# CODEJIN/GST_Tacotron

Measured on AMD Instinct MI355X. Metric: mel-frames/s, higher is better.
Workload: dtype f32; 1 GPU; BASELINE configs[1]: GST on, batch 32 per GPU, 128-token utterances, Step_Reduction 2, Max_Step 1000, LJSpeech 80-mel hparams; whole Inference_Step (encoder+GST+decode+postnet, vocoder excluded); global_batch=32, ref_frames=256, parallelism=utterance-sharded x1 + final RCCL gather, gather=none (one rank)

## Files before the change

gst_tacotron_amd/capi.py:

```python
import ctypes
import os

import numpy as np
import torch

from .hparams import Dims

_HERE = os.path.dirname(os.path.abspath(__file__))
LIB_PATH = os.path.join(_HERE, "lib", "libgsttaco.so")

MAX_LAYERS = 8
ABI_VERSION = 13
ATT_CODES = {"BMA": 0, "SMA": 1, "LSA": 2}

EXPORTED_SYMBOLS = (
    "gsttaco_abi_version", "gsttaco_create", "gsttaco_destroy", "gsttaco_last_error",
    "gsttaco_num_weights", "gsttaco_weight_info", "gsttaco_load_weight", "gsttaco_finalize_weights",
    "gsttaco_encode", "gsttaco_gst", "gsttaco_decode", "gsttaco_postnet", "gsttaco_vocoder", "gsttaco_inference_step",
    "gsttaco_mel_frontend", "gsttaco_mel_basis", "gsttaco_griffin_lim", "gsttaco_crc32c",
    "gsttaco_set_profiling", "gsttaco_get_profile", "gsttaco_lstm_launch_bytes", "gsttaco_debug_stamps", "gsttaco_decode_plan", "gsttaco_debug_randomness",
    "gsttaco_set_graph_policy", "gsttaco_graph_cache_size", "gsttaco_debug_handoff_error", "gsttaco_debug_raise_handoff_error", "gsttaco_debug_counters",
    "gsttaco_synchronize", "gsttaco_debug_conv_prepare", "gsttaco_debug_conv_run",
)

CONV_V = {
    "IG_1411": 0, "IG_2212": 1, "IG_2222": 2, "IG_4113": 3, "IG_4112": 4, "IG_4111": 5,
    "C2D_1411": 6, "C2D_4112": 7, "C2D_4111": 8,
    "WINO4": 9, "WINO2": 10, "WINO4_S": 11, "WINO2_S": 12, "WINO4_S_X3": 13, "WINO2_S_X3": 14,
    "GEMM_SPLIT": 15,
    "C5_RN4": 16, "C5_RN4_XB": 17, "C5_RN4_OB": 18, "C5_RN4_XB_OB": 19,
    "C5_RN2": 20, "C5_RN2_XB": 21, "C5_RN2_OB": 22, "C5_RN2_XB_OB": 23,
    "BF16_RM2": 24, "BF16_RM2_XB": 25, "BF16_RM2_OB": 26, "BF16_RM2_XB_OB": 27,
    "BF16_RM1": 28, "BF16_RM1_XB": 29, "BF16_RM1_OB": 30, "BF16_RM1_XB_OB": 31,
}
CONV_V_INVALID = -1
CONV_V_NAMES = {v: k for k, v in CONV_V.items()}
CONV_FORM = {"FP32": 1, "BF16": 2, "WINO2": 4, "WINO4": 8, "WINO_SPLIT": 16, "GEMM_SPLIT": 32}
# ... 78 lines not shown
    lib.gsttaco_decode.argtypes = [vp, vp, vp, vp, vp, vp, u64, i32, i32, i32, vp, vp, vp, vp]
    lib.gsttaco_postnet.argtypes = [vp, vp, i32, i32, vp, vp]
    lib.gsttaco_vocoder.argtypes = [vp, vp, i32, i32, vp, vp]
    lib.gsttaco_inference_step.argtypes = [vp, vp, vp, vp, vp, vp, vp, u64, i32, i32, i32, i32, vp, vp, vp, vp, vp, vp]
    lib.gsttaco_mel_frontend.argtypes = [vp, vp, vp, i32, i32, ctypes.c_float, vp, vp, i32, vp]
    lib.gsttaco_mel_basis.argtypes = [vp, f32p]
    lib.gsttaco_griffin_lim.argtypes = [vp, vp, vp, i32, i32, i32, ctypes.c_float, ctypes.c_float, vp, u64, vp, vp, i32, vp]
    lib.gsttaco_set_profiling.argtypes = [vp, i32]
    lib.gsttaco_get_profile.argtypes = [vp, i32, ctypes.POINTER(ctypes.c_float), ctypes.POINTER(ctypes.c_int)]
    lib.gsttaco_lstm_launch_bytes.argtypes = [vp, i32, i32]
    lib.gsttaco_lstm_launch_bytes.restype = ctypes.c_int64
    lib.gsttaco_debug_stamps.argtypes = [vp, ctypes.POINTER(ctypes.c_uint64)]
    lib.gsttaco_debug_stamps.restype = ctypes.c_int
    lib.gsttaco_decode_plan.argtypes = [vp, i32, ctypes.POINTER(ctypes.c_int32)]
    lib.gsttaco_decode_plan.restype = ctypes.c_int
    lib.gsttaco_debug_randomness.argtypes = [vp, vp, vp, i32, i32, i32]
    lib.gsttaco_debug_randomness.restype = ctypes.c_int
    lib.gsttaco_set_graph_policy.argtypes = [vp, i32, i32]
    lib.gsttaco_set_graph_policy.restype = ctypes.c_int
    lib.gsttaco_graph_cache_size.argtypes = [vp]
    lib.gsttaco_graph_cache_size.restype = ctypes.c_int
    lib.gsttaco_debug_handoff_error.argtypes = [vp, ctypes.POINTER(ctypes.c_uint32)]
    lib.gsttaco_debug_handoff_error.restype = ctypes.c_int
    lib.gsttaco_debug_raise_handoff_error.argtypes = [vp, ctypes.c_uint32]
    lib.gsttaco_debug_raise_handoff_error.restype = ctypes.c_int
    lib.gsttaco_debug_counters.argtypes = [vp, ctypes.POINTER(ctypes.c_uint64)]
    lib.gsttaco_debug_counters.restype = ctypes.c_int
    lib.gsttaco_synchronize.argtypes = [vp, vp]
    lib.gsttaco_synchronize.restype = ctypes.c_int
    lib.gsttaco_debug_conv_prepare.argtypes = [vp, ctypes.POINTER(ConvDesc), f32p, f32p, f32p, ctypes.POINTER(ctypes.c_int)]
# ... 116 lines not shown
```

gst_tacotron_amd/csrc/gsttaco.cpp:

```cpp
#include <hip/hip_runtime.h>

#include <algorithm>
#include <atomic>
#include <cmath>
#include <cstdio>
#include <cstdlib>
#include <cstring>
#include <map>
#include <mutex>
#include <string>
#include <vector>

#include "../../include/gsttaco.h"
#include "kernels.h"

namespace {

constexpr float kBnEps = 1e-3f;

struct HostTensor {
    std::string name;
    std::vector<int64_t> shape;
    std::vector<float> data;
    bool loaded = false;
// ... 2399 lines not shown
    }
    const uint8_t* p = static_cast<const uint8_t*>(data);
    uint32_t c = crc ^ 0xffffffffu;
    while (n >= 8) {
        uint32_t lo, hi;
        memcpy(&lo, p, 4); memcpy(&hi, p + 4, 4);
        lo ^= c;
        c = tab[7][lo & 0xff] ^ tab[6][(lo >> 8) & 0xff] ^ tab[5][(lo >> 16) & 0xff] ^ tab[4][lo >> 24] ^
            tab[3][hi & 0xff] ^ tab[2][(hi >> 8) & 0xff] ^ tab[1][(hi >> 16) & 0xff] ^ tab[0][hi >> 24];
        p += 8; n -= 8;
    }
    while (n--) c = tab[0][(c ^ *p++) & 0xff] ^ (c >> 8);
    return c ^ 0xffffffffu;
}

int gsttaco_debug_randomness(gsttaco_ctx* c, float* host_masks, float* host_noise, int steps, int B, int Tv) {
    if (!c || steps < 1 || B < 1 || Tv < 1 || steps > c->steps_max || B > c->cfg.max_batch || Tv > c->cfg.max_tokens)
        return GSTTACO_E_INVALID;
    HIPCHECK(c, hipDeviceSynchronize());
    if (host_masks && c->masks_lazy) {
        HIPCHECK(c, gt_launch_rng_fill(c->w_seed, c->w_masks, nullptr, steps, B, c->P0, c->P1, Tv, c->cfg.prenet_rate, nullptr));
        HIPCHECK(c, hipDeviceSynchronize());
    }
    if (host_masks && c->dec_padded) {
        float* tmp = nullptr;
        const size_t n = (size_t)steps * B * (c->P0t + c->P1t);
        HIPCHECK(c, hipMalloc((void**)&tmp, n * 4));
        hipError_t e = gt_launch_relayout_masks(c->w_masks, tmp, steps, B, c->P0t, c->P1t, c->P0, c->P1, 0, nullptr);
        if (e == hipSuccess) e = hipMemcpy(host_masks, tmp, n * 4, hipMemcpyDeviceToHost);
        (void)hipFree(tmp);
// ... 116 lines not shown
```

gst_tacotron_amd/csrc/kernels.h:

```cpp
#pragma once
#include <hip/hip_runtime.h>
#include <stdint.h>

enum { EPI_LINEAR = 0, EPI_RELU_DROP = 1, EPI_LSTM = 2, EPI_PARTIAL = 3 };

struct SkinnySeg {
    const float* ptr;
    int64_t ld;
    int nkb;
    int blocked;
};
__host__ __device__ inline size_t gt_blk_off(int row, int k, int MT) {
    return (((size_t)(k >> 4) * MT + (row >> 4)) << 8) + (size_t)(((((k & 15) >> 2) << 4) + (row & 15)) * 4 + (k & 3));
}

__host__ __device__ inline size_t gt_blk_off_h(int row, int k, int MT) {
    return ((((size_t)(k >> 5) * MT + (row >> 4)) << 6) + (size_t)((((k & 15) >> 2) << 4) + (row & 15))) * 8 + (size_t)((((k >> 4) & 1) << 2) + (k & 3));
}

struct SkinnyArgs {
    const float* wp;
    const float* bias;
    SkinnySeg seg[3];
    int nkb;
// ... 256 lines not shown
    float* hpart;
    float* stash;
    uint32_t* ctl;
    uint32_t* err;
    float* pre; int64_t ld_pre;
    float* stop;
    float* align; int64_t ld_align;
    int B, MT, Tv, steps, co_tiles;
    int G, n_chain, tvp, twopass;
    int expect_extra;
    unsigned long long* dbg;
};
size_t gt_persist_decode_ctl_words();
bool gt_persist_decode_supported(int mel, int r, int P0, int P1, int A, int H1, int H2, int B, int Tv, int pj_tiles, int pj_nkb, int slots, int bf16);
int gt_persist_decode_max_batch();
bool gt_persist_decode_lsa_fits(int B, int Tv, int loc_f, int loc_k);
hipError_t gt_persist_decode_init();
int gt_persist_decode_blocks_per_cu();
hipError_t gt_launch_persist_decode(const PersistDecodeArgs& a, const float* b0, hipStream_t stream);

struct Conv2dArgs {
    const float* x;
    int64_t xb;
    const float* w;
    const float* scale;
    const float* shift;
    float* out;
    int B, H, W, Cin, Cout, Ho, Wo, k, stride, pad_h, pad_w;
};
hipError_t gt_launch_conv2d_bn_relu(const Conv2dArgs& a, hipStream_t stream);
// ... 59 lines not shown
```

gst_tacotron_amd/csrc/persist_decode.hip:

```cpp
#include "chain_common.h"
#include "device_utils.h"
#include "kernels.h"
#include "../../include/gsttaco.h"

namespace {

constexpr int PD_NT = 512, PD_NW = 8, PD_NWG = 256, PD_UTT = 32, PD_HELP = 64;
constexpr int PD_P = 256, PD_A = 128, PD_H = 1024, PD_TVMAX = 256, PD_LDV = PD_A + 4;
constexpr int PD_GMAX = 4, PD_BMAX = 32 * PD_GMAX;
constexpr int PD_KBP = PD_P / 16, PD_KBC = PD_A / 16, PD_KBH = PD_H / 16, PD_KBPJ = PD_KBH + PD_KBC;
constexpr uint32_t PD_SPIN_MAX = 1u << 20;

#ifndef PD_FS
#define PD_FS 16
#endif
#ifndef PD_SLEEP_N
#define PD_SLEEP_N 0
#endif
#define PD_SLEEP() do { if (PD_SLEEP_N > 0) __builtin_amdgcn_s_sleep(PD_SLEEP_N); } while (0)
#define PD_ZT(zt) int zt = 0; asm volatile("" : "+v"(zt))
#ifndef PD_X2_EARLY
#define PD_X2_EARLY 1
#endif
#ifndef PD_NSH
#define PD_NSH 64
#endif
constexpr int PD_F_P = 0, PD_F_C = PD_BMAX * 32, PD_CNT3 = 2 * PD_BMAX * 32, PD_CNT4 = PD_CNT3 + PD_GMAX * PD_NSH * 32,
              PD_F_H = PD_CNT4 + PD_GMAX * PD_NSH * 32, PD_CTL_WORDS = PD_F_H + 128 * 32;

__device__ __forceinline__ uint32_t pd_ld_sc1(const uint32_t* p) {
    uint32_t v;
    asm volatile("global_load_dword %0, %1, off sc1\n\ts_waitcnt vmcnt(0)" : "=v"(v) : "v"(p) : "memory");
    return v;
}
__device__ __forceinline__ uint2 pd_ld2_sc1(const uint2* p) {
    uint2 v;
    asm volatile("global_load_dwordx2 %0, %1, off sc1\n\ts_waitcnt vmcnt(0)" : "=v"(v) : "v"(p) : "memory");
    return v;
}
__device__ __forceinline__ void pd_st4_sc1(float* p, float4 v) {
    f32x4 t = {v.x, v.y, v.z, v.w};
    asm volatile("global_store_dwordx4 %0, %1, off sc1" ::"v"(p), "v"(t) : "memory");
}
__device__ __forceinline__ void pd_st2_sc1(uint2* p, uint2 v) { asm volatile("global_store_dwordx2 %0, %1, off sc1" ::"v"(p), "v"(v) : "memory"); }
__device__ __forceinline__ void pd_st1_sc1(uint32_t* p, uint32_t v) { asm volatile("global_store_dword %0, %1, off sc1" ::"v"(p), "v"(v) : "memory"); }
__device__ __forceinline__ void pd_drain() { asm volatile("s_waitcnt vmcnt(0)" ::: "memory"); }

#define PD_PIN() do { asm volatile("" ::: "memory"); __builtin_amdgcn_sched_barrier(0); } while (0)
#define PD_PIN4(a) do { asm volatile("" : "+v"((a).x), "+v"((a).y), "+v"((a).z), "+v"((a).w) : : "memory"); __builtin_amdgcn_sched_barrier(0); } while (0)

struct PdShared { int abort; };
#define PD_PHASE_ABORT(sh) do { } while (0)
#define PD_HOLD(p)                                                                                      \
    do {                                                                                                \
        const uint64_t u_ = reinterpret_cast<uint64_t>(p);                                              \
        uint32_t lo_ = __builtin_amdgcn_readfirstlane((uint32_t)u_), hi_ = __builtin_amdgcn_readfirstlane((uint32_t)(u_ >> 32)); \
        asm volatile("" : "+s"(lo_), "+s"(hi_));                                                        \
        p = reinterpret_cast<decltype(p)>(((uint64_t)hi_ << 32) | lo_);                                 \
    } while (0)

#define PD_STAMP(role, slot)                                                                                              \
    do {                                                                                                                  \
        if (A.dbg && t == (A.steps >> 1) && threadIdx.x == 0 && (blockIdx.x == 0 || (int)blockIdx.x == A.n_chain || blockIdx.x == PD_NWG - 1)) \
            A.dbg[(role) * 32 + (slot)] = __builtin_amdgcn_s_memrealtime();                                                 \
    } while (0)

// ... 34 lines not shown
            bool ok = uf >= fwant;
#pragma unroll
            for (int k = 0; k < PD_NSH / 64; ++k) { asm volatile("" : "+v"(u[k])); ok = ok && u[k] >= want; }
            if (__builtin_amdgcn_readfirstlane(__popcll(__ballot(ok))) == 64) break;
            if (++spins > PD_SPIN_MAX) { if (lane == 0) pd_give_up(A, sh, true); break; }
            if ((spins & 63u) == 0u && __builtin_amdgcn_readfirstlane(pd_ld_sc1(A.err)) != 0u) { if (lane == 0) pd_give_up(A, sh, false); break; }
            PD_SLEEP();
        }
    }
    __syncthreads();
}
__device__ __forceinline__ void pd_arrive(uint32_t* c) {
    pd_drain();
    __syncthreads();
    if (threadIdx.x == 0) __hip_atomic_fetch_add(c + (blockIdx.x & (PD_NSH - 1)) * 32, 1u, __ATOMIC_RELAXED, __HIP_MEMORY_SCOPE_AGENT);
}

template <int I0, int I1, int NB>
__device__ __forceinline__ void pd_xload(const float* base, int MT, float4 (&x0)[NB], float4 (&x1)[NB]) {
    const int lane = threadIdx.x & 63;
    const int wave = __builtin_amdgcn_readfirstlane(threadIdx.x >> 6);
    const auto rs = gt_rsrc(base, 0x7FFFF000u);
    const uint32_t m1 = (uint32_t)min(1, MT - 1) * 1024u;
#pragma unroll
    for (int i = I0; i < I1; ++i) {
        const uint32_t so = (uint32_t)((wave + i * PD_NW) * MT) * 1024u;
        x0[i] = gt_bload4_sc1(rs, (uint32_t)lane * 16u, so);
        x1[i] = gt_bload4_sc1(rs, (uint32_t)lane * 16u, so + m1);
    }
}
// ... 162 lines not shown
        PD_PIN();
        pd_mma<1, 2, 1, 3>(x0, x1, W.x1, a0, a1);
    } else {
        pd_wait_flags<PD_FS>(A, A.ctl + PD_F_C, A.B, (uint32_t)t + 1u, sh);
        PD_PHASE_ABORT(sh);
        PD_STAMP(role, 3);
        pd_xload<0, 3, 3>(xa, MT, x0, x1);
        if (stream_x2) { int tz = tile; asm volatile("" : "+s"(tz)); pd_load_tile<8>(A.w2x, tz, W.x2); }
        PD_PIN();
        pd_mma<3, 0, 1, 3>(x0, x1, W.x1, a0, a1);
    }
    pd_spill(lds, threadIdx.x >> 6, a0, a1);
    const float z = pd_reduce<8, false>(lds, p1v);
    pd_gates_store(z, c1v, h1d, tile, A.B, MT);
    PD_STAMP(role, 4);
    pd_arrive(A.ctl + PD_CNT3);
}

__device__ __forceinline__ void pd_cell2(const PersistDecodeArgs& A, PdW& W, int t, int tile, float* lds, float& c2v, float& p2v, float& p1_next, bool with_rec1,
                                        PdShared* sh, int help_tile, bool stream_h1, bool stream_x2, int role = 2, int helped_p2 = -1, bool helped_role = false) {
    const int par = t & 1, MT = A.MT;
    float4 wu[8];
    if (help_tile >= 0) pd_load_tile<8>(A.w1h, help_tile, wu);
    if (stream_h1) pd_load_tile<8>(A.w1h, tile, W.h1);
    const float* h1p = A.h1[par];
    float* h2d = A.h2[par];
    PD_HOLD(h1p); PD_HOLD(h2d);
    pd_wait_count(A, A.ctl + PD_CNT3, PD_WANT(A, t), sh, helped_p2 >= 0 ? A.ctl + PD_F_H + helped_p2 * 32 : nullptr, (uint32_t)t);
    PD_PHASE_ABORT(sh);
    PD_STAMP(role, 5);
    float4 x0[8], x1[8];
    if (stream_x2) pd_load_tile<8>(A.w2x, tile, W.x2);
    pd_xload<0, 8, 8>(h1p, MT, x0, x1);
    float4 d2 = make_float4(0.f, 0.f, 0.f, 0.f);
    if (helped_role) {
        const auto rh = gt_rsrc(A.hpart, 2u * 32u * 512u * 4u);
        d2 = gt_bload4_sc1(rh, helped_p2 >= 0 ? (uint32_t)((helped_p2 * 512 + ((int)threadIdx.x & ~3)) * 4) : GT_OOB, 0u);
    }
    PD_PIN();
    PD_STAMP(role, 21);
    f32x4 a0 = {0, 0, 0, 0}, a1 = {0, 0, 0, 0};
    pd_mma<8, 0, 1, 8>(x0, x1, W.x2, a0, a1);
    PD_STAMP(role, 6);
    if (helped_role && helped_p2 >= 0) {
        const int e = threadIdx.x & 3;
        p2v = e == 0 ? d2.x : e == 1 ? d2.y : e == 2 ? d2.z : d2.w;
    }
    pd_spill(lds, threadIdx.x >> 6, a0, a1);
    const float z = pd_reduce<8, false>(lds, p2v);
    PD_STAMP(role, 22);
    pd_gates_store(z, c2v, h2d, tile, A.B, MT);
    PD_STAMP(role, 7);
    pd_arrive(A.ctl + PD_CNT4);
    PD_STAMP(role, 8);
    const int col = threadIdx.x & 15;
    if (help_tile >= 0) {
        const float v = pd_rec_tile<true>(x0, x1, wu, A.b1h[help_tile * 16 + col], lds);
        pd_publish_part(v, A.hpart + (size_t)help_tile * 512, A.ctl + PD_F_H + help_tile * 32, (uint32_t)t + 1u);
    }
    if (with_rec1) p1_next = pd_rec_tile<true>(x0, x1, W.h1, A.b1h[tile * 16 + col], lds);
}

__device__ __forceinline__ float pd_rec2(const PersistDecodeArgs& A, int t, const float* hbuf, const float4 (&wh)[8], int tile, int help_tile, float* lds) {
    float4 wu[8];
    if (help_tile >= 0) pd_load_tile<8>(A.w2h, help_tile, wu);
    float4 x0[8], x1[8];
    pd_xload<0, 8, 8>(hbuf, A.MT, x0, x1);
    PD_PIN();
    const int col = threadIdx.x & 15;
    if (help_tile >= 0) {
        const float v = help_tile < A.co_tiles ? pd_rec_tile<false>(x0, x1, wu, A.b2h[help_tile * 16 + col], lds)
                                               : pd_rec_tile<true>(x0, x1, wu, A.b2h[help_tile * 16 + col], lds);
        pd_publish_part(v, A.hpart + (size_t)(32 + help_tile) * 512, A.ctl + PD_F_H + (32 + help_tile) * 32, (uint32_t)t + 1u);
    }
    return tile < A.co_tiles ? pd_rec_tile<false>(x0, x1, wh, A.b2h[tile * 16 + col], lds) : pd_rec_tile<true>(x0, x1, wh, A.b2h[tile * 16 + col], lds);
}
__device__ __forceinline__ float pd_rec1_mem(const PersistDecodeArgs& A, const float* hbuf, const float4 (&wh)[8], int tile, float* lds) {
    float4 x0[8], x1[8];
    pd_xload<0, 8, 8>(hbuf, A.MT, x0, x1);
    PD_PIN();
    return pd_rec_tile<true>(x0, x1, wh, A.b1h[tile * 16 + (threadIdx.x & 15)], lds);
}

template <bool GK = false>
__device__ __forceinline__ void pd_proj(const PersistDecodeArgs& A, const float4 (&wp)[9], int t, int ptile, int pmt, float* lds, PdShared* sh, int g = 0) {
    const int par = t & 1, MT = A.MT;
    const float* h2p = A.h2[par];
    const float* xap = A.xa[par];
    uint2* z0g = A.z0g;
    PD_HOLD(h2p); PD_HOLD(xap); PD_HOLD(z0g);
    if (!GK) {
        pd_wait_count(A, A.ctl + PD_CNT4, PD_WANT(A, t), sh);
        PD_PHASE_ABORT(sh);
    }
    if (!GK) PD_STAMP(1, 9);
    const int lane = threadIdx.x & 63;
    const int wave = __builtin_amdgcn_readfirstlane(threadIdx.x >> 6);
    const auto rh = gt_rsrc(h2p, 0x7FFFF000u);
    const auto rx = gt_rsrc(xap, 0x7FFFF000u);
    float4 x[9];
#pragma unroll
    for (int i = 0; i < 9; ++i) {
        const int kb = wave + i * PD_NW;
        x[i] = kb < PD_KBH ? gt_bload4_sc1(rh, (uint32_t)lane * 16u, (uint32_t)((kb * MT + pmt) * 1024))
                           : gt_bload4_sc1(rx, (uint32_t)lane * 16u, (uint32_t)(((kb - PD_KBH + PD_KBP) * MT + pmt) * 1024));
    }
    PD_PIN();
    f32x4 a0 = {0, 0, 0, 0}, a1 = {0, 0, 0, 0};
#pragma unroll
    for (int i = 0; i < 9; ++i) {
        a0 = __builtin_amdgcn_mfma_f32_16x16x4f32(x[i].x, wp[i].x, a0, 0, 0, 0);
        a0 = __builtin_amdgcn_mfma_f32_16x16x4f32(x[i].y, wp[i].y, a0, 0, 0, 0);
        a0 = __builtin_amdgcn_mfma_f32_16x16x4f32(x[i].z, wp[i].z, a0, 0, 0, 0);
        a0 = __builtin_amdgcn_mfma_f32_16x16x4f32(x[i].w, wp[i].w, a0, 0, 0, 0);
    }
    if (!GK) PD_STAMP(1, 10);
    pd_spill(lds, threadIdx.x >> 6, a0, a1);
    const float v = GK ? pd_reduce<8>(lds, A.bp[ptile * 16 + (threadIdx.x & 15)]) : pd_reduce<8, false>(lds, A.bp[ptile * 16 + (threadIdx.x & 15)]);
    const int row = threadIdx.x >> 4, col = threadIdx.x & 15;
    const int grow = pmt * 16 + row, gcol = ptile * 16 + col;
    if (row < 16 && grow < A.B) {
        if (gcol >= A.z_col0) {
            if (gcol < A.z_col0 + PD_P) {
                uint2 g;
                g.x = __builtin_bit_cast(uint32_t, v); g.y = (uint32_t)t + 1u;
                pd_st2_sc1(z0g + (size_t)grow * PD_P + (gcol - A.z_col0), g);
            }
        } else if (gcol < A.n_split) {
            A.pre[(size_t)grow * A.ld_pre + (size_t)t * A.n_split + gcol] = v;
        } else if (gcol < A.n_out) {
            A.stop[(size_t)grow * A.steps + t] = v;
        }
    }
    if (!GK) PD_STAMP(1, 11);
// ... 403 lines not shown
    PD_STAMP(0, 20);
}

template <bool HELPED, bool MIRROR = false, bool TV128 = false, bool LSA = false>
__device__ __forceinline__ void pd_chain(const PersistDecodeArgs& A, const PdChainLds& L, const PdChainRegs& R, int t, int b, PdShared* sh, float4& hraw, int zt = 0) {
    float4 ra[16], rb[16];
    pd_chain_issue(A, R, t, b, zt, ra, rb);
    pd_chain_rest<HELPED, MIRROR, TV128, LSA>(A, L, R, t, b, sh, hraw, zt, ra, rb);
}

__device__ __forceinline__ void pd_run_chain(const PersistDecodeArgs& A, float* smem, PdShared* sh) {
    float* lds = smem;
    PdChainLds L = pd_carve(smem, A.tvp);
    const bool lsa = A.att_type == GSTTACO_ATT_LSA;
    if (lsa) L.lpack = L.lfeat + 128 * gt_lsa_pack(PD_A, A.loc_f, A.loc_k).LFS;
    const int tile = blockIdx.x, b = blockIdx.x, tid = threadIdx.x, col = tid & 15;
    const bool live = b < A.B;
    PdW W;
    float c1v = 0.f, c2v = 0.f, p1v = A.b1h[tile * 16 + col], p2v = A.b2h[tile * 16 + col];
    PdChainRegs R{};
    if (live) {
        R.Tv = A.tok_len ? max(1, min(A.Tv, (int)A.tok_len[b])) : A.Tv;
        R.drop = A.drop_rate > 0.f;
        R.hashed = R.drop && A.keep_hash != 0;
        R.noisy = A.sigmoid_noise > 0.f;
        R.seed = R.hashed ? *A.seed_ptr : 0ull;
        R.bias1 = tid < PD_P ? A.b1[tid] : 0.f;
        R.biasq = tid < PD_A ? A.bq[tid] : 0.f;
        R.sbias = lsa ? 0.f : A.score_bias[0];
        const float4* src = reinterpret_cast<const float4*>(A.pm + (size_t)b * A.Tv * PD_A);
        for (int e = tid; e < A.tvp * PD_A / 4; e += PD_NT) {
// ... 13 lines not shown
        PD_STAMP(0, 0);
        if (A.dbg && threadIdx.x == 0 && blockIdx.x == 0) {
            const int ts[8] = {0, 1, 2, 8, 64, A.steps >> 1, (3 * A.steps) >> 2, A.steps - 1};
#pragma unroll
            for (int k = 0; k < 8; ++k) if (t == ts[k]) A.dbg[24 + k] = __builtin_amdgcn_s_memrealtime();
        }
        if (live) {
            PD_ZT(zt);
            float4 hraw;
            if (lsa) pd_chain<true, false, true, true>(A, L, R, t, b, sh, hraw, zt);
            else if (A.tvp == 128) pd_chain<true, false, true>(A, L, R, t, b, sh, hraw, zt);
            else pd_chain<true>(A, L, R, t, b, sh, hraw, zt);
            PD_PHASE_ABORT(sh);
            if (t > 0) { const int e = tid & 3; p1v = e == 0 ? hraw.x : e == 1 ? hraw.y : e == 2 ? hraw.z : hraw.w; }
        } else if (t > 0) {
            pd_wait_flags(A, A.ctl + PD_F_H + tile * 32, 1, (uint32_t)t, sh);
            PD_PHASE_ABORT(sh);
            const auto rh = gt_rsrc(A.hpart, 2u * 32u * 512u * 4u);
            const float4 d1 = gt_bload4_sc1(rh, (uint32_t)((tile * 512 + (tid & ~3)) * 4), 0u);
            const int e = tid & 3;
            p1v = e == 0 ? d1.x : e == 1 ? d1.y : e == 2 ? d1.z : d1.w;
        }
        pd_cell1(A, W, t, tile, lds, c1v, p1v, sh, false, true, 0, PD_X2_EARLY != 0);
        PD_PHASE_ABORT(sh);
        float unused = 0.f;
        pd_cell2(A, W, t, tile, lds, c2v, p2v, unused, false, sh, -1, false, PD_X2_EARLY == 0, 0, t > 0 ? 32 + tile : -1, true);
        PD_PHASE_ABORT(sh);
    }
}

__device__ __forceinline__ void pd_run_proj(const PersistDecodeArgs& A, float* lds, PdShared* sh) {
    const int tile = blockIdx.x, col = threadIdx.x & 15;
    const int pi = tile - PD_UTT, ptile = pi % A.pj_tiles, pmt = pi / A.pj_tiles;
    PdW W;
    pd_load_tile<3>(A.w1x, tile, W.x1); pd_load_tile<8>(A.w2x, tile, W.x2);
    float4 wpj[9];
    pd_load_tile<9>(A.wp, ptile, wpj);
    float c1v = 0.f, c2v = 0.f, p1v = A.b1h[tile * 16 + col], p2v = A.b2h[tile * 16 + col];
    for (int t = 0; t < A.steps; ++t) {
        if (sh->abort) return;
        const int par = t & 1;
        PD_STAMP(1, 0);
        pd_cell1(A, W, t, tile, lds, c1v, p1v, sh, true, false, 1);
        PD_PHASE_ABORT(sh);
        float unused = 0.f;
        pd_cell2(A, W, t, tile, lds, c2v, p2v, unused, false, sh, -1, false, false, 1);
        PD_PHASE_ABORT(sh);
        pd_proj(A, wpj, t, ptile, pmt, lds, sh);
        PD_PHASE_ABORT(sh);
        if (t + 1 == A.steps) break;
        pd_load_tile<8>(A.w1h, tile, W.h1);
        PD_PIN();
        p1v = pd_rec1_mem(A, A.h1[par], W.h1, tile, lds);
        pd_load_tile<8>(A.w2h, tile, W.h2);
        PD_PIN();
        p2v = pd_rec2(A, t, A.h2[par], W.h2, tile, -1, lds);
    }
}

template <int HELP>
__device__ __forceinline__ void pd_run_plain(const PersistDecodeArgs& A, float* lds, PdShared* sh, int help_tile) {
    const int tile = blockIdx.x, col = threadIdx.x & 15;
    PdW W;
    pd_load_tile<3>(A.w1x, tile, W.x1); pd_load_tile<8>(A.w2x, tile, W.x2);
    if (HELP != 2) pd_load_tile<8>(A.w1h, tile, W.h1);
    if (HELP != 1) pd_load_tile<8>(A.w2h, tile, W.h2);
    float c1v = 0.f, c2v = 0.f, p1v = A.b1h[tile * 16 + col], p2v = A.b2h[tile * 16 + col];
    for (int t = 0; t < A.steps; ++t) {
        if (sh->abort) return;
        const int par = t & 1;
        PD_STAMP(2, 0);
        pd_cell1(A, W, t, tile, lds, c1v, p1v, sh, true);
        PD_PHASE_ABORT(sh);
        pd_cell2(A, W, t, tile, lds, c2v, p2v, p1v, true, sh, HELP == 1 ? help_tile : -1, HELP == 2, false);
        PD_STAMP(2, 12);
        PD_PHASE_ABORT(sh);
        if (t + 1 == A.steps) break;
        if (HELP == 1) pd_load_tile<8>(A.w2h, tile, W.h2);
        pd_wait_count(A, A.ctl + PD_CNT4, PD_WANT(A, t), sh);
        PD_PHASE_ABORT(sh);
        PD_STAMP(2, 13);
        p2v = pd_rec2(A, t, A.h2[par], W.h2, tile, HELP == 2 ? help_tile : -1, lds);
        PD_STAMP(2, 14);
    }
}

__global__ __launch_bounds__(PD_NT) void gt_persist_decode_kernel(PersistDecodeArgs A) {
    extern __shared__ __attribute__((aligned(16))) float smem[];
    __shared__ PdShared sh;
    if (threadIdx.x == 0) sh.abort = 0;
    if (A.dbg && threadIdx.x == 0 && (blockIdx.x == 0 || blockIdx.x == PD_NWG - 1)) A.dbg[blockIdx.x == 0 ? 9 : 10] = __builtin_amdgcn_s_memrealtime();
    __syncthreads();
    const int tile = blockIdx.x;
    const int n_pj = A.pj_tiles * A.MT;
#ifndef PD_ONLY
#define PD_ONLY -1
#endif
    if (tile < PD_UTT) { if (PD_ONLY < 0 || PD_ONLY == 0) pd_run_chain(A, smem, &sh); }
    else if (tile < PD_UTT + n_pj) { if (PD_ONLY < 0 || PD_ONLY == 1) pd_run_proj(A, smem, &sh); }
    else {
        const int hidx = tile - (PD_UTT + n_pj);
        if (hidx >= PD_HELP) { if (PD_ONLY < 0 || PD_ONLY == 2) pd_run_plain<0>(A, smem, &sh, -1); }
        else if ((hidx & 1) == 0) { if (PD_ONLY < 0 || PD_ONLY == 3) pd_run_plain<1>(A, smem, &sh, hidx >> 1); }
        else if (PD_ONLY < 0 || PD_ONLY == 4) pd_run_plain<2>(A, smem, &sh, hidx >> 1);
    }
// ... 7 lines not shown
    const int i = blockIdx.x * blockDim.x + threadIdx.x;
    if (i < PD_CTL_WORDS) ctl[i] = 0u;
    if (i < B * PD_P) {
        uint2 g;
        g.x = __builtin_bit_cast(uint32_t, b0[i % PD_P]); g.y = 0u;
        z0g[i] = g;
    }
}

}

size_t gt_persist_decode_ctl_words() { return PD_CTL_WORDS; }

int gt_persist_decode_max_batch() { return PD_BMAX; }

bool gt_persist_decode_lsa_fits(int B, int Tv, int loc_f, int loc_k) {
    return B <= 32 && Tv <= 128 && loc_f >= 1 && loc_k >= 1 && pd_lds_floats(128) + pd_lsa_floats(loc_f, loc_k) <= pd_lds_floats(PD_TVMAX, true);
}

__host__ __device__ constexpr int pdh_chain_floats(int tvp, int nslab) { return nslab * PDH_SLAB + 3 * PD_P + 2 * PD_A + 4 * tvp + tvp * PD_LDV; }
__host__ __device__ constexpr int pdh_chain_slabs(int) { return 8; }
__host__ __device__ constexpr int pdh_lds_floats(int tvp) {
    return pdh_chain_floats(tvp, pdh_chain_slabs(tvp)) > 16 * PDH_SLAB ? pdh_chain_floats(tvp, pdh_chain_slabs(tvp)) : 16 * PDH_SLAB;
}
constexpr int PDH_TVMAX = 192;
static_assert(pdh_lds_floats(PDH_TVMAX) * 4 + 64 <= 160 * 1024, "the bf16 kernel's chain state must fit a CU's LDS");

bool gt_persist_decode_supported(int mel, int r, int P0, int P1, int A, int H1, int H2, int B, int Tv, int pj_tiles, int pj_nkb, int slots, int bf16) {
    (void)mel; (void)r;
    if (!(P0 == PD_P && P1 == PD_P && A == PD_A && H1 == PD_H && H2 == PD_H && B >= 1 && Tv >= 1 && Tv <= PD_TVMAX && pj_nkb == PD_KBPJ && pj_tiles >= 1 &&
// ... 37 lines not shown
    if (a.bf16) {
        a.G = 1;
        a.tvp = (a.Tv + 63) / 64 * 64;
        a.n_chain = a.B;
        a.twopass = 0;
        const int n = PD_CTL_WORDS > a.B * PD_P ? PD_CTL_WORDS : a.B * PD_P;
        hipLaunchKernelGGL(gt_persist_decode_init_kernel, dim3((n + 255) / 256), dim3(256), 0, stream, a.z0g, b0, a.ctl, a.B);
        hipLaunchKernelGGL(gt_persist_decode_h_kernel, dim3(PD_NWG), dim3(PD_NT), (size_t)pdh_lds_floats(a.tvp) * 4, stream, a);
        return hipGetLastError();
    }
    const bool lsa = a.att_type == GSTTACO_ATT_LSA;
    const PdKernel k = pd_kernel_for(a.B, &a.G);
    a.tvp = lsa ? 128 : (a.Tv + 63) / 64 * 64;
    const bool gk = k != gt_persist_decode_kernel;
    if (lsa && (gk || !gt_persist_decode_lsa_fits(a.B, a.Tv, a.loc_f, a.loc_k))) return hipErrorInvalidValue;
    a.n_chain = gk ? a.B : PD_UTT;
    a.twopass = pd_chain_slabs(a.tvp, gk) == 8 ? 1 : 0;
    const int n = PD_CTL_WORDS > a.B * PD_P ? PD_CTL_WORDS : a.B * PD_P;
    hipLaunchKernelGGL(gt_persist_decode_init_kernel, dim3((n + 255) / 256), dim3(256), 0, stream, a.z0g, b0, a.ctl, a.B);
    hipLaunchKernelGGL(k, dim3(PD_NWG), dim3(PD_NT), (size_t)(pd_lds_floats(a.tvp, gk) + (lsa ? pd_lsa_floats(a.loc_f, a.loc_k) : 0)) * 4, stream, a);
    return hipGetLastError();
}
```

include/gsttaco.h:

```cpp
#ifndef GSTTACO_H
#define GSTTACO_H

#include <stddef.h>
#include <stdint.h>

#ifdef __cplusplus
extern "C" {
#endif

#define GSTTACO_ABI_VERSION 13
#define GSTTACO_MAX_LAYERS 8

enum {
    GSTTACO_OK = 0,
    GSTTACO_E_INVALID = -1,
    GSTTACO_E_NO_DEVICE = -2,
    GSTTACO_E_HIP = -3,
    GSTTACO_E_WEIGHTS = -4,
    GSTTACO_E_CAPACITY = -5
};

enum { GSTTACO_ATT_BMA = 0, GSTTACO_ATT_SMA = 1, GSTTACO_ATT_LSA = 2 };

typedef struct gsttaco_config {
// ... 96 lines not shown

int gsttaco_mel_basis(gsttaco_ctx* ctx, float* host_out);

int gsttaco_inference_step(gsttaco_ctx* ctx, const int32_t* tokens, const int32_t* token_lengths,
                           const float* mels_for_gst, const int32_t* mel_lengths,
                           const float* prenet_mask, const float* attn_noise, uint64_t seed,
                           int B, int Tv, int Tref1, int steps,
                           float* mel, float* stop, float* align, float* pre_mel, float* spectrogram, void* stream);

int gsttaco_set_graph_policy(gsttaco_ctx* ctx, int max_cached, int capture_after);
int gsttaco_graph_cache_size(const gsttaco_ctx* ctx);

int gsttaco_set_profiling(gsttaco_ctx* ctx, int every);
int gsttaco_get_profile(gsttaco_ctx* ctx, int layer, float* avg_ms, int* count);
int gsttaco_debug_stamps(gsttaco_ctx* ctx, unsigned long long* host_out96);
int gsttaco_synchronize(gsttaco_ctx* ctx, void* stream);
int gsttaco_debug_handoff_error(gsttaco_ctx* ctx, uint32_t* host_out);
int gsttaco_debug_counters(const gsttaco_ctx* ctx, uint64_t out[4]);
int gsttaco_debug_raise_handoff_error(gsttaco_ctx* ctx, uint32_t bits);
int gsttaco_debug_randomness(gsttaco_ctx* ctx, float* host_masks, float* host_noise, int steps, int B, int Tv);
int gsttaco_decode_plan(const gsttaco_ctx* ctx, int Tv, int32_t plan[3]);
int64_t gsttaco_lstm_launch_bytes(const gsttaco_ctx* ctx, int layer, int B);

enum {
    GSTTACO_CONV_V_INVALID = -1,
    GSTTACO_CONV_V_IG_1411 = 0, GSTTACO_CONV_V_IG_2212 = 1, GSTTACO_CONV_V_IG_2222 = 2,
    GSTTACO_CONV_V_IG_4113 = 3, GSTTACO_CONV_V_IG_4112 = 4, GSTTACO_CONV_V_IG_4111 = 5,
    GSTTACO_CONV_V_C2D_1411 = 6, GSTTACO_CONV_V_C2D_4112 = 7, GSTTACO_CONV_V_C2D_4111 = 8,
    GSTTACO_CONV_V_WINO4 = 9, GSTTACO_CONV_V_WINO2 = 10,
    GSTTACO_CONV_V_WINO4_S = 11, GSTTACO_CONV_V_WINO2_S = 12, GSTTACO_CONV_V_WINO4_S_X3 = 13, GSTTACO_CONV_V_WINO2_S_X3 = 14,
// ... 33 lines not shown
```

Baseline: 3.098 million mel-frames/s.

## Split persistent decode barriers into shard and chain-line counters with optional two-stage wait

Chain workgroups now arrive on dedicated chain-line counters instead of the sharded counters, and workgroup-to-tile mapping is rotated so the chain groups own the last tiles. The waits check both counter sets. An optional two-stage mode, off by default, lets cell2 and the projection start on the early K-blocks once the non-chain shards arrive, and wait for the chain counters only before the final blocks. The goal is to shorten barrier latency on the critical recurrent path, at the cost of extra polling and more complex control-word layout. A debug export that reports the per-workgroup plan is also added.

```diff
diff --git a/gst_tacotron_amd/capi.py b/gst_tacotron_amd/capi.py
--- a/gst_tacotron_amd/capi.py
+++ b/gst_tacotron_amd/capi.py
@@ -20,7 +20,7 @@
     "gsttaco_mel_frontend", "gsttaco_mel_basis", "gsttaco_griffin_lim", "gsttaco_crc32c",
     "gsttaco_set_profiling", "gsttaco_get_profile", "gsttaco_lstm_launch_bytes", "gsttaco_debug_stamps", "gsttaco_decode_plan", "gsttaco_debug_randomness",
     "gsttaco_set_graph_policy", "gsttaco_graph_cache_size", "gsttaco_debug_handoff_error", "gsttaco_debug_raise_handoff_error", "gsttaco_debug_counters",
-    "gsttaco_synchronize", "gsttaco_debug_conv_prepare", "gsttaco_debug_conv_run",
+    "gsttaco_synchronize", "gsttaco_debug_conv_prepare", "gsttaco_debug_conv_run", "gsttaco_debug_persist_plan",
 )
 
 CONV_V = {
@@ -129,6 +129,8 @@
     lib.gsttaco_debug_stamps.restype = ctypes.c_int
     lib.gsttaco_decode_plan.argtypes = [vp, i32, ctypes.POINTER(ctypes.c_int32)]
     lib.gsttaco_decode_plan.restype = ctypes.c_int
+    lib.gsttaco_debug_persist_plan.argtypes = [i32, i32, i32, ctypes.POINTER(ctypes.c_int32 * 5)]
+    lib.gsttaco_debug_persist_plan.restype = ctypes.c_int
     lib.gsttaco_debug_randomness.argtypes = [vp, vp, vp, i32, i32, i32]
     lib.gsttaco_debug_randomness.restype = ctypes.c_int
     lib.gsttaco_set_graph_policy.argtypes = [vp, i32, i32]
diff --git a/gst_tacotron_amd/csrc/gsttaco.cpp b/gst_tacotron_amd/csrc/gsttaco.cpp
--- a/gst_tacotron_amd/csrc/gsttaco.cpp
+++ b/gst_tacotron_amd/csrc/gsttaco.cpp
@@ -2437,6 +2437,13 @@
     return c ^ 0xffffffffu;
 }
 
+int gsttaco_debug_persist_plan(int batch, int pj_tiles, int wg, int32_t out[5]) {
+    PersistDecodePlan p;
+    if (!out || !gt_persist_decode_plan(batch, pj_tiles, wg, &p)) return GSTTACO_E_INVALID;
+    out[0] = p.role; out[1] = p.tile; out[2] = p.line3; out[3] = p.line4; out[4] = p.help;
+    return 0;
+}
+
 int gsttaco_debug_randomness(gsttaco_ctx* c, float* host_masks, float* host_noise, int steps, int B, int Tv) {
     if (!c || steps < 1 || B < 1 || Tv < 1 || steps > c->steps_max || B > c->cfg.max_batch || Tv > c->cfg.max_tokens)
         return GSTTACO_E_INVALID;
diff --git a/gst_tacotron_amd/csrc/kernels.h b/gst_tacotron_amd/csrc/kernels.h
--- a/gst_tacotron_amd/csrc/kernels.h
+++ b/gst_tacotron_amd/csrc/kernels.h
@@ -294,6 +294,8 @@
 size_t gt_persist_decode_ctl_words();
 bool gt_persist_decode_supported(int mel, int r, int P0, int P1, int A, int H1, int H2, int B, int Tv, int pj_tiles, int pj_nkb, int slots, int bf16);
 int gt_persist_decode_max_batch();
+struct PersistDecodePlan { int role, tile, line3, line4, help; };
+bool gt_persist_decode_plan(int B, int pj_tiles, int wg, PersistDecodePlan* out);
 bool gt_persist_decode_lsa_fits(int B, int Tv, int loc_f, int loc_k);
 hipError_t gt_persist_decode_init();
 int gt_persist_decode_blocks_per_cu();
diff --git a/gst_tacotron_amd/csrc/persist_decode.hip b/gst_tacotron_amd/csrc/persist_decode.hip
--- a/gst_tacotron_amd/csrc/persist_decode.hip
+++ b/gst_tacotron_amd/csrc/persist_decode.hip
@@ -25,8 +25,21 @@
 #ifndef PD_NSH
 #define PD_NSH 64
 #endif
+constexpr int PD_CPL = PD_NWG / PD_NSH, PD_NCL = PD_UTT / PD_CPL;
 constexpr int PD_F_P = 0, PD_F_C = PD_BMAX * 32, PD_CNT3 = 2 * PD_BMAX * 32, PD_CNT4 = PD_CNT3 + PD_GMAX * PD_NSH * 32,
-              PD_F_H = PD_CNT4 + PD_GMAX * PD_NSH * 32, PD_CTL_WORDS = PD_F_H + 128 * 32;
+              PD_F_H = PD_CNT4 + PD_GMAX * PD_NSH * 32, PD_CNT3C = PD_F_H + 128 * 32,
+              PD_CNT4C = PD_CNT3C + PD_NCL * 32, PD_CTL_WORDS = PD_CNT4C + PD_NCL * 32;
+static_assert(PD_UTT % PD_CPL == 0 && PD_NCL <= 64 && PD_NSH >= PD_UTT, "whole chain lines, one per lane; a shard loses at most one arrival to them");
+
+__host__ __device__ constexpr int pd_tile_of(int wg) { return (wg + PD_NWG - PD_UTT) % PD_NWG; }
+__host__ __device__ constexpr int pd_line_of(int wg) { return wg < PD_UTT ? PD_NSH + wg / PD_CPL : (wg & (PD_NSH - 1)); }
+__host__ __device__ constexpr int pd_shard_arrivals(int s) { return PD_CPL - (s < PD_UTT ? 1 : 0); }
+#ifndef PD_TWO_STAGE
+#define PD_TWO_STAGE 0
+#endif
+#ifndef PD_S2_K
+#define PD_S2_K 6
+#endif
 
 __device__ __forceinline__ uint32_t pd_ld_sc1(const uint32_t* p) {
     uint32_t v;
@@ -49,7 +62,7 @@
 #define PD_PIN() do { asm volatile("" ::: "memory"); __builtin_amdgcn_sched_barrier(0); } while (0)
 #define PD_PIN4(a) do { asm volatile("" : "+v"((a).x), "+v"((a).y), "+v"((a).z), "+v"((a).w) : : "memory"); __builtin_amdgcn_sched_barrier(0); } while (0)
 
-struct PdShared { int abort; };
+struct PdShared { int abort; uint32_t st2; };
 #define PD_PHASE_ABORT(sh) do { } while (0)
 #define PD_HOLD(p)                                                                                      \
     do {                                                                                                \
@@ -114,6 +127,67 @@
     pd_drain();
     __syncthreads();
     if (threadIdx.x == 0) __hip_atomic_fetch_add(c + (blockIdx.x & (PD_NSH - 1)) * 32, 1u, __ATOMIC_RELAXED, __HIP_MEMORY_SCOPE_AGENT);
+}
+
+__device__ __forceinline__ void pd_arrive2(uint32_t* c, uint32_t* cc) {
+    pd_drain();
+    __syncthreads();
+    if (threadIdx.x == 0)
+        __hip_atomic_fetch_add(blockIdx.x < PD_UTT ? cc + (blockIdx.x / PD_CPL) * 32 : c + (blockIdx.x & (PD_NSH - 1)) * 32, 1u, __ATOMIC_RELAXED, __HIP_MEMORY_SCOPE_AGENT);
+}
+template <bool BOTH>
+__device__ __forceinline__ bool pd_wait_stage1(const PersistDecodeArgs& A, const uint32_t* c, const uint32_t* cc, int t, uint32_t tag, PdShared* sh,
+                                               const uint32_t* flag = nullptr, uint32_t fwant = 0u) {
+    static_assert(PD_NSH == 64, "one counter shard per lane");
+    if (threadIdx.x < 64) {
+        const int lane = threadIdx.x;
+        const uint32_t want1 = (uint32_t)(t + 1) * (uint32_t)pd_shard_arrivals(lane) + (uint32_t)A.expect_extra;
+        const uint32_t want2 = (uint32_t)(t + 1) * (uint32_t)PD_CPL + (uint32_t)A.expect_extra;
+        const int voff = lane * 128;
+        uint32_t spins = 0;
+        for (;;) {
+            uint32_t uf = fwant;
+            asm volatile("" ::: "memory");
+            const uint32_t u = __builtin_amdgcn_raw_buffer_load_b32(gt_rsrc(c, (uint32_t)(PD_NSH * 32 * 4)), voff, 0, 16);
+            uint32_t v = __builtin_amdgcn_raw_buffer_load_b32(gt_rsrc(cc, (uint32_t)(PD_NCL * 32 * 4)), voff, 0, 16);
+            if (flag) uf = __builtin_amdgcn_raw_buffer_load_b32(gt_rsrc(flag, 4u), 0, 0, 16);
+            if (lane >= PD_NCL) v = want2;
+            const bool a1 = __builtin_amdgcn_readfirstlane(__popcll(__ballot(u >= want1 && uf >= fwant))) == 64;
+            const bool a2 = __builtin_amdgcn_readfirstlane(__popcll(__ballot(v >= want2))) == 64;
+            if (a1 && (!BOTH || a2)) { if (!BOTH && a2 && lane == 0) sh->st2 = tag; break; }
+            if (++spins > PD_SPIN_MAX) { if (lane == 0) pd_give_up(A, sh, true); break; }
+            if ((spins & 63u) == 0u && __builtin_amdgcn_readfirstlane(pd_ld_sc1(A.err)) != 0u) { if (lane == 0) pd_give_up(A, sh, false); break; }
+            PD_SLEEP();
+        }
+    }
+    __syncthreads();
+    if (BOTH) return true;
+    return __builtin_amdgcn_readfirstlane((int)(sh->st2 == tag)) != 0;
+}
+__device__ __forceinline__ uint32_t pd_stage2_poll(const uint32_t* cc) {
+    uint32_t v = 0u;
+    if (__builtin_amdgcn_readfirstlane(threadIdx.x >> 6) == 0)
+        v = __builtin_amdgcn_raw_buffer_load_b32(gt_rsrc(cc, (uint32_t)(PD_NCL * 32 * 4)), (int)((threadIdx.x & 63u) * 128u), 0, 16);
+    return v;
+}
+__device__ __forceinline__ void pd_stage2_join(const PersistDecodeArgs& A, const uint32_t* cc, int t, uint32_t tag, PdShared* sh, uint32_t v) {
+    volatile uint32_t* st = &sh->st2;
+    if (__builtin_amdgcn_readfirstlane(threadIdx.x >> 6) == 0) {
+        const int lane = threadIdx.x & 63;
+        const uint32_t want2 = (uint32_t)(t + 1) * (uint32_t)PD_CPL + (uint32_t)A.expect_extra;
+        uint32_t spins = 0;
+        for (;;) {
+            if (__builtin_amdgcn_readfirstlane(__popcll(__ballot(lane >= PD_NCL || v >= want2))) == 64) break;
+            if (++spins > PD_SPIN_MAX) { if (lane == 0) pd_give_up(A, sh, true); break; }
+            if ((spins & 63u) == 0u && __builtin_amdgcn_readfirstlane(pd_ld_sc1(A.err)) != 0u) { if (lane == 0) pd_give_up(A, sh, false); break; }
+            PD_SLEEP();
+            asm volatile("" ::: "memory");
+            v = __builtin_amdgcn_raw_buffer_load_b32(gt_rsrc(cc, (uint32_t)(PD_NCL * 32 * 4)), (int)((uint32_t)lane * 128u), 0, 16);
+        }
+        if (lane == 0) *st = tag;
+    } else {
+        while (*st != tag) __builtin_amdgcn_s_sleep(1);
+    }
 }
 
 template <int I0, int I1, int NB>
@@ -306,11 +380,12 @@
     const float z = pd_reduce<8, false>(lds, p1v);
     pd_gates_store(z, c1v, h1d, tile, A.B, MT);
     PD_STAMP(role, 4);
-    pd_arrive(A.ctl + PD_CNT3);
+    pd_arrive2(A.ctl + PD_CNT3, A.ctl + PD_CNT3C);
 }
 
 __device__ __forceinline__ void pd_cell2(const PersistDecodeArgs& A, PdW& W, int t, int tile, float* lds, float& c2v, float& p2v, float& p1_next, bool with_rec1,
-                                        PdShared* sh, int help_tile, bool stream_h1, bool stream_x2, int role = 2, int helped_p2 = -1, bool helped_role = false) {
+                                        PdShared* sh, int help_tile, bool stream_h1, bool stream_x2, int role = 2, int helped_p2 = -1, bool helped_role = false,
+                                        int help_idx = -1) {
     const int par = t & 1, MT = A.MT;
     float4 wu[8];
     if (help_tile >= 0) pd_load_tile<8>(A.w1h, help_tile, wu);
@@ -318,12 +393,17 @@
     const float* h1p = A.h1[par];
     float* h2d = A.h2[par];
     PD_HOLD(h1p); PD_HOLD(h2d);
-    pd_wait_count(A, A.ctl + PD_CNT3, PD_WANT(A, t), sh, helped_p2 >= 0 ? A.ctl + PD_F_H + helped_p2 * 32 : nullptr, (uint32_t)t);
+    const uint32_t tag = 2u * (uint32_t)t + 1u;
+    const bool early = pd_wait_stage1<PD_TWO_STAGE == 0>(A, A.ctl + PD_CNT3, A.ctl + PD_CNT3C, t, tag, sh, helped_p2 >= 0 ? A.ctl + PD_F_H + helped_p2 * 32 : nullptr, (uint32_t)t);
     PD_PHASE_ABORT(sh);
     PD_STAMP(role, 5);
     float4 x0[8], x1[8];
     if (stream_x2) pd_load_tile<8>(A.w2x, tile, W.x2);
-    pd_xload<0, 8, 8>(h1p, MT, x0, x1);
+    pd_xload<0, PD_S2_K, 8>(h1p, MT, x0, x1);
+    uint32_t s2v = 0u;
+    if (!early) s2v = pd_stage2_poll(A.ctl + PD_CNT3C);
+    pd_xload<PD_S2_K, 7, 8>(h1p, MT, x0, x1);
+    if (early) pd_xload<7, 8, 8>(h1p, MT, x0, x1);
     float4 d2 = make_float4(0.f, 0.f, 0.f, 0.f);
     if (helped_role) {
         const auto rh = gt_rsrc(A.hpart, 2u * 32u * 512u * 4u);
@@ -332,7 +412,14 @@
     PD_PIN();
     PD_STAMP(role, 21);
     f32x4 a0 = {0, 0, 0, 0}, a1 = {0, 0, 0, 0};
-    pd_mma<8, 0, 1, 8>(x0, x1, W.x2, a0, a1);
+    pd_mma<PD_S2_K, 0, 1, 8>(x0, x1, W.x2, a0, a1);
+    if (!early) {
+        pd_stage2_join(A, A.ctl + PD_CNT3C, t, tag, sh, s2v);
+        PD_STAMP(role, role == 0 ? 11 : 24);
+        pd_xload<7, 8, 8>(h1p, MT, x0, x1);
+        PD_PIN();
+    }
+    pd_mma<8 - PD_S2_K, PD_S2_K, 1, 8>(x0, x1, W.x2, a0, a1);
     PD_STAMP(role, 6);
     if (helped_role && helped_p2 >= 0) {
         const int e = threadIdx.x & 3;
@@ -343,17 +430,17 @@
     PD_STAMP(role, 22);
     pd_gates_store(z, c2v, h2d, tile, A.B, MT);
     PD_STAMP(role, 7);
-    pd_arrive(A.ctl + PD_CNT4);
+    pd_arrive2(A.ctl + PD_CNT4, A.ctl + PD_CNT4C);
     PD_STAMP(role, 8);
     const int col = threadIdx.x & 15;
     if (help_tile >= 0) {
         const float v = pd_rec_tile<true>(x0, x1, wu, A.b1h[help_tile * 16 + col], lds);
-        pd_publish_part(v, A.hpart + (size_t)help_tile * 512, A.ctl + PD_F_H + help_tile * 32, (uint32_t)t + 1u);
+        pd_publish_part(v, A.hpart + (size_t)help_idx * 512, A.ctl + PD_F_H + help_idx * 32, (uint32_t)t + 1u);
     }
     if (with_rec1) p1_next = pd_rec_tile<true>(x0, x1, W.h1, A.b1h[tile * 16 + col], lds);
 }
 
-__device__ __forceinline__ float pd_rec2(const PersistDecodeArgs& A, int t, const float* hbuf, const float4 (&wh)[8], int tile, int help_tile, float* lds) {
+__device__ __forceinline__ float pd_rec2(const PersistDecodeArgs& A, int t, const float* hbuf, const float4 (&wh)[8], int tile, int help_tile, float* lds, int help_idx = -1) {
     float4 wu[8];
     if (help_tile >= 0) pd_load_tile<8>(A.w2h, help_tile, wu);
     float4 x0[8], x1[8];
@@ -363,7 +450,7 @@
     if (help_tile >= 0) {
         const float v = help_tile < A.co_tiles ? pd_rec_tile<false>(x0, x1, wu, A.b2h[help_tile * 16 + col], lds)
                                                : pd_rec_tile<true>(x0, x1, wu, A.b2h[help_tile * 16 + col], lds);
-        pd_publish_part(v, A.hpart + (size_t)(32 + help_tile) * 512, A.ctl + PD_F_H + (32 + help_tile) * 32, (uint32_t)t + 1u);
+        pd_publish_part(v, A.hpart + (size_t)(32 + help_idx) * 512, A.ctl + PD_F_H + (32 + help_idx) * 32, (uint32_t)t + 1u);
     }
     return tile < A.co_tiles ? pd_rec_tile<false>(x0, x1, wh, A.b2h[tile * 16 + col], lds) : pd_rec_tile<true>(x0, x1, wh, A.b2h[tile * 16 + col], lds);
 }
@@ -381,8 +468,10 @@
     const float* xap = A.xa[par];
     uint2* z0g = A.z0g;
     PD_HOLD(h2p); PD_HOLD(xap); PD_HOLD(z0g);
+    const uint32_t tag = 2u * (uint32_t)t + 2u;
+    bool early = true;
     if (!GK) {
-        pd_wait_count(A, A.ctl + PD_CNT4, PD_WANT(A, t), sh);
+        early = pd_wait_stage1<PD_TWO_STAGE == 0>(A, A.ctl + PD_CNT4, A.ctl + PD_CNT4C, t, tag, sh);
         PD_PHASE_ABORT(sh);
     }
     if (!GK) PD_STAMP(1, 9);
@@ -391,9 +480,12 @@
     const auto rh = gt_rsrc(h2p, 0x7FFFF000u);
     const auto rx = gt_rsrc(xap, 0x7FFFF000u);
     float4 x[9];
+    uint32_t s2v = 0u;
 #pragma unroll
     for (int i = 0; i < 9; ++i) {
         const int kb = wave + i * PD_NW;
+        if (!GK && i == PD_S2_K && !early) s2v = pd_stage2_poll(A.ctl + PD_CNT4C);
+        if (!GK && i == 7 && !early) continue;
         x[i] = kb < PD_KBH ? gt_bload4_sc1(rh, (uint32_t)lane * 16u, (uint32_t)((kb * MT + pmt) * 1024))
                            : gt_bload4_sc1(rx, (uint32_t)lane * 16u, (uint32_t)(((kb - PD_KBH + PD_KBP) * MT + pmt) * 1024));
     }
@@ -401,6 +493,12 @@
     f32x4 a0 = {0, 0, 0, 0}, a1 = {0, 0, 0, 0};
 #pragma unroll
     for (int i = 0; i < 9; ++i) {
+        if (!GK && i == PD_S2_K && !early) {
+            pd_stage2_join(A, A.ctl + PD_CNT4C, t, tag, sh, s2v);
+            PD_STAMP(1, 25);
+            x[7] = gt_bload4_sc1(rh, (uint32_t)lane * 16u, (uint32_t)(((wave + 7 * PD_NW) * MT + pmt) * 1024));
+            PD_PIN();
+        }
         a0 = __builtin_amdgcn_mfma_f32_16x16x4f32(x[i].x, wp[i].x, a0, 0, 0, 0);
         a0 = __builtin_amdgcn_mfma_f32_16x16x4f32(x[i].y, wp[i].y, a0, 0, 0, 0);
         a0 = __builtin_amdgcn_mfma_f32_16x16x4f32(x[i].z, wp[i].z, a0, 0, 0, 0);
@@ -409,7 +507,9 @@
     if (!GK) PD_STAMP(1, 10);
     pd_spill(lds, threadIdx.x >> 6, a0, a1);
     const float v = GK ? pd_reduce<8>(lds, A.bp[ptile * 16 + (threadIdx.x & 15)]) : pd_reduce<8, false>(lds, A.bp[ptile * 16 + (threadIdx.x & 15)]);
-    const int row = threadIdx.x >> 4, col = threadIdx.x & 15;
+    int zr = 0;
+    if (!GK) asm volatile("" : "+v"(zr));
+    const int row = (int)(threadIdx.x >> 4) + zr, col = threadIdx.x & 15;
     const int grow = pmt * 16 + row, gcol = ptile * 16 + col;
     if (row < 16 && grow < A.B) {
         if (gcol >= A.z_col0) {
@@ -843,7 +943,7 @@
     PdChainLds L = pd_carve(smem, A.tvp);
     const bool lsa = A.att_type == GSTTACO_ATT_LSA;
     if (lsa) L.lpack = L.lfeat + 128 * gt_lsa_pack(PD_A, A.loc_f, A.loc_k).LFS;
-    const int tile = blockIdx.x, b = blockIdx.x, tid = threadIdx.x, col = tid & 15;
+    const int tile = pd_tile_of(blockIdx.x), b = blockIdx.x, tid = threadIdx.x, col = tid & 15;
     const bool live = b < A.B;
     PdW W;
     float c1v = 0.f, c2v = 0.f, p1v = A.b1h[tile * 16 + col], p2v = A.b2h[tile * 16 + col];
@@ -887,24 +987,24 @@
             PD_PHASE_ABORT(sh);
             if (t > 0) { const int e = tid & 3; p1v = e == 0 ? hraw.x : e == 1 ? hraw.y : e == 2 ? hraw.z : hraw.w; }
         } else if (t > 0) {
-            pd_wait_flags(A, A.ctl + PD_F_H + tile * 32, 1, (uint32_t)t, sh);
+            pd_wait_flags(A, A.ctl + PD_F_H + b * 32, 1, (uint32_t)t, sh);
             PD_PHASE_ABORT(sh);
             const auto rh = gt_rsrc(A.hpart, 2u * 32u * 512u * 4u);
-            const float4 d1 = gt_bload4_sc1(rh, (uint32_t)((tile * 512 + (tid & ~3)) * 4), 0u);
+            const float4 d1 = gt_bload4_sc1(rh, (uint32_t)((b * 512 + (tid & ~3)) * 4), 0u);
             const int e = tid & 3;
             p1v = e == 0 ? d1.x : e == 1 ? d1.y : e == 2 ? d1.z : d1.w;
         }
         pd_cell1(A, W, t, tile, lds, c1v, p1v, sh, false, true, 0, PD_X2_EARLY != 0);
         PD_PHASE_ABORT(sh);
         float unused = 0.f;
-        pd_cell2(A, W, t, tile, lds, c2v, p2v, unused, false, sh, -1, false, PD_X2_EARLY == 0, 0, t > 0 ? 32 + tile : -1, true);
+        pd_cell2(A, W, t, tile, lds, c2v, p2v, unused, false, sh, -1, false, PD_X2_EARLY == 0, 0, t > 0 ? 32 + b : -1, true);
         PD_PHASE_ABORT(sh);
     }
 }
 
 __device__ __forceinline__ void pd_run_proj(const PersistDecodeArgs& A, float* lds, PdShared* sh) {
-    const int tile = blockIdx.x, col = threadIdx.x & 15;
-    const int pi = tile - PD_UTT, ptile = pi % A.pj_tiles, pmt = pi / A.pj_tiles;
+    const int tile = pd_tile_of(blockIdx.x), col = threadIdx.x & 15;
+    const int pi = (int)blockIdx.x - PD_UTT, ptile = pi % A.pj_tiles, pmt = pi / A.pj_tiles;
     PdW W;
     pd_load_tile<3>(A.w1x, tile, W.x1); pd_load_tile<8>(A.w2x, tile, W.x2);
     float4 wpj[9];
@@ -932,8 +1032,9 @@
 }
 
 template <int HELP>
-__device__ __forceinline__ void pd_run_plain(const PersistDecodeArgs& A, float* lds, PdShared* sh, int help_tile) {
-    const int tile = blockIdx.x, col = threadIdx.x & 15;
+__device__ __forceinline__ void pd_run_plain(const PersistDecodeArgs& A, float* lds, PdShared* sh, int help_idx) {
+    const int tile = pd_tile_of(blockIdx.x), col = threadIdx.x & 15;
+    const int help_tile = help_idx >= 0 ? pd_tile_of(help_idx) : -1;
     PdW W;
     pd_load_tile<3>(A.w1x, tile, W.x1); pd_load_tile<8>(A.w2x, tile, W.x2);
     if (HELP != 2) pd_load_tile<8>(A.w1h, tile, W.h1);
@@ -945,15 +1046,15 @@
         PD_STAMP(2, 0);
         pd_cell1(A, W, t, tile, lds, c1v, p1v, sh, true);
         PD_PHASE_ABORT(sh);
-        pd_cell2(A, W, t, tile, lds, c2v, p2v, p1v, true, sh, HELP == 1 ? help_tile : -1, HELP == 2, false);
+        pd_cell2(A, W, t, tile, lds, c2v, p2v, p1v, true, sh, HELP == 1 ? help_tile : -1, HELP == 2, false, 2, -1, false, help_idx);
         PD_STAMP(2, 12);
         PD_PHASE_ABORT(sh);
         if (t + 1 == A.steps) break;
         if (HELP == 1) pd_load_tile<8>(A.w2h, tile, W.h2);
-        pd_wait_count(A, A.ctl + PD_CNT4, PD_WANT(A, t), sh);
+        pd_wait_stage1<true>(A, A.ctl + PD_CNT4, A.ctl + PD_CNT4C, t, 0u, sh);
         PD_PHASE_ABORT(sh);
         PD_STAMP(2, 13);
-        p2v = pd_rec2(A, t, A.h2[par], W.h2, tile, HELP == 2 ? help_tile : -1, lds);
+        p2v = pd_rec2(A, t, A.h2[par], W.h2, tile, HELP == 2 ? help_tile : -1, lds, help_idx);
         PD_STAMP(2, 14);
     }
 }
@@ -961,7 +1062,7 @@
 __global__ __launch_bounds__(PD_NT) void gt_persist_decode_kernel(PersistDecodeArgs A) {
     extern __shared__ __attribute__((aligned(16))) float smem[];
     __shared__ PdShared sh;
-    if (threadIdx.x == 0) sh.abort = 0;
+    if (threadIdx.x == 0) { sh.abort = 0; sh.st2 = 0u; }
     if (A.dbg && threadIdx.x == 0 && (blockIdx.x == 0 || blockIdx.x == PD_NWG - 1)) A.dbg[blockIdx.x == 0 ? 9 : 10] = __builtin_amdgcn_s_memrealtime();
     __syncthreads();
     const int tile = blockIdx.x;
@@ -999,6 +1100,20 @@
 
 int gt_persist_decode_max_batch() { return PD_BMAX; }
 
+bool gt_persist_decode_plan(int B, int pj_tiles, int wg, PersistDecodePlan* out) {
+    if (B < 1 || B > 32 || pj_tiles < 1 || wg < 0 || wg >= PD_NWG || !out) return false;
+    const int n_pj = pj_tiles * ((B + 15) / 16);
+    if (PD_UTT + n_pj + PD_HELP > PD_NWG) return false;
+    const int hidx = wg - (PD_UTT + n_pj);
+    out->role = wg < PD_UTT ? 0 : hidx < 0 ? 1 : hidx >= PD_HELP ? 2 : 3 + (hidx & 1);
+    out->tile = pd_tile_of(wg);
+    const int line = pd_line_of(wg);
+    out->line3 = line < PD_NSH ? PD_CNT3 / 32 + line : PD_CNT3C / 32 + (line - PD_NSH);
+    out->line4 = line < PD_NSH ? PD_CNT4 / 32 + line : PD_CNT4C / 32 + (line - PD_NSH);
+    out->help = out->role >= 3 ? hidx >> 1 : -1;
+    return true;
+}
+
 bool gt_persist_decode_lsa_fits(int B, int Tv, int loc_f, int loc_k) {
     return B <= 32 && Tv <= 128 && loc_f >= 1 && loc_k >= 1 && pd_lds_floats(128) + pd_lsa_floats(loc_f, loc_k) <= pd_lds_floats(PD_TVMAX, true);
 }
@@ -1066,6 +1181,18 @@
     a.tvp = lsa ? 128 : (a.Tv + 63) / 64 * 64;
     const bool gk = k != gt_persist_decode_kernel;
     if (lsa && (gk || !gt_persist_decode_lsa_fits(a.B, a.Tv, a.loc_f, a.loc_k))) return hipErrorInvalidValue;
+    if (!gk) {
+        static const bool plan_ok = [] {
+            bool seen[PD_NWG] = {}, ok = true;
+            for (int w = 0; w < PD_NWG; ++w) {
+                const int tl = pd_tile_of(w);
+                ok = ok && !seen[tl] && (w < PD_UTT) == (tl >= PD_NWG - PD_UTT) && (w < PD_UTT) == (pd_line_of(w) >= PD_NSH);
+                seen[tl] = true;
+            }
+            return ok;
+        }();
+        if (!plan_ok) return hipErrorInvalidValue;
+    }
     a.n_chain = gk ? a.B : PD_UTT;
     a.twopass = pd_chain_slabs(a.tvp, gk) == 8 ? 1 : 0;
     const int n = PD_CTL_WORDS > a.B * PD_P ? PD_CTL_WORDS : a.B * PD_P;
diff --git a/include/gsttaco.h b/include/gsttaco.h
--- a/include/gsttaco.h
+++ b/include/gsttaco.h
@@ -134,6 +134,7 @@
 int gsttaco_set_profiling(gsttaco_ctx* ctx, int every);
 int gsttaco_get_profile(gsttaco_ctx* ctx, int layer, float* avg_ms, int* count);
 int gsttaco_debug_stamps(gsttaco_ctx* ctx, unsigned long long* host_out96);
+int gsttaco_debug_persist_plan(int batch, int pj_tiles, int wg, int32_t out[5]);
 int gsttaco_synchronize(gsttaco_ctx* ctx, void* stream);
 int gsttaco_debug_handoff_error(gsttaco_ctx* ctx, uint32_t* host_out);
 int gsttaco_debug_counters(const gsttaco_ctx* ctx, uint64_t out[4]);
```

Result: slower. 2.985 million mel-frames/s (-3.7%).
